# lijun9250lj/video-steganography-PCAMV

Hardware: AMD Instinct MI355X
Metric: 1080p macroblocks/s (embed on) (higher is better)
Workload: dtype u8

## Files before the change

### video-steganography-pcamv_amd/csrc/pcamv_common.h

```cpp
#ifndef PCAMV_COMMON_H
#define PCAMV_COMMON_H
#include <stddef.h>
#include <stdint.h>
#include "../../include/pcamv_gpu.h"
#include "pcamv_variant.h"

#ifdef PCAMV_HOST_EMU
#define PCAMV_DEV static inline
#define PCAMV_CONST static const
#else
#include <hip/hip_runtime.h>
#define PCAMV_DEV __device__ __forceinline__
#define PCAMV_CONST __device__ static const
#endif

#define PCAMV_PAD 32
#define PCAMV_CPAD 16
#define PCAMV_LSW 28
#define PCAMV_LROW 32
#define PCAMV_LSTRIPS(stride) (((stride) + PCAMV_LSW - 1) / PCAMV_LSW + 1)
#define PCAMV_LSTRIP_OF(x) (((uint32_t)(x) * 18725u) >> 19)
#define PCAMV_COST_MAX (1 << 28)
#define PCAMV_COST_MV_LEN (4 * 4 * 2048 + 1)
#define PCAMV_COST_MV_CENTRE (2 * 4 * 2048)
// ... 14 lines not shown
    uint8_t *luma[4];
    uint8_t *chroma[2];
    uint8_t *rec[3];
    int8_t *mb_type;
    int16_t *mv;
    int8_t *ref8;
    int16_t *mvr;
    const int16_t *prev_mv;
    const int8_t *prev_ref;
    int have_prev, tscale;
    pcamv_mb_t *rec_mb;
    int16_t *mvp_aux;
    const int16_t *cost_mv;
    int qp, chroma_qp, lambda, chroma_qp_offset;
    int me_method, me_range, subme, mv_range, b_chroma_me, b_fast_pskip, b_dct_decimate, b_cabac;
    unsigned inter;
    int embed;
    int q_mf[2][3], q_bias[2][3], dq_mf[3];
    int dq_mf_c[3];
    int lambda2_chroma;
    int *trace; int trace_mb;
    uint16_t *nnz;
    const int8_t *flip;
    const int *car_base;
    int b_mbrd, psy_rd, lambda2, ref_is_inter;
    int q_mf_i[3], q_bias_i[3];
    uint8_t *nb_nz;
    int16_t *nb_cbp;
    int16_t *nb_mvd;
    uint8_t *cabac;
    const uint8_t *cabac_init;
    const uint32_t *cabac_tab;
    uint32_t *dbg_hash;
    int rec_is_pass1;
    const uint8_t *mbflip;
    const struct FrameDev *self;
};

#ifdef PCAMV_HOST_EMU
#define FD(F) (F)
#else
#define PCAMV_AS4 __attribute__((address_space(4)))
PCAMV_DEV const PCAMV_AS4 FrameDev &fd_reload(const FrameDev &F)
{
    const uint64_t a = (uint64_t)F.self;
    uint32_t lo = (uint32_t)__builtin_amdgcn_readfirstlane((int)(uint32_t)a), hi = (uint32_t)__builtin_amdgcn_readfirstlane((int)(uint32_t)(a >> 32));
    asm volatile("" : "+s"(lo), "+s"(hi));
    return *(const PCAMV_AS4 FrameDev *)((uint64_t)hi << 32 | lo);
}
template <bool KEEP> PCAMV_DEV const auto &fd_pick(const FrameDev &F) { if constexpr (KEEP) return F; else return fd_reload(F); }
#ifdef PCAMV_NO_DESC_RELOAD
#define FD(F) (F)
#else
#define FD(F) fd_pick<PCAMV_RD_LO>(F)
#endif
#endif

PCAMV_DEV int nib32(unsigned k, int i) { return (int)((k >> (4 * i)) & 15u); }
PCAMV_DEV int nib64(unsigned long long k, int i) { return (int)((k >> (4 * i)) & 15ull); }
PCAMV_DEV int lg_w4_of(int ip) { return nib32(0x0011122u, ip); }
PCAMV_DEV int lg_h4_of(int ip) { return nib32(0x0101212u, ip); }
PCAMV_DEV int lg_nblk_of(int ip) { return nib32(0x0112334u, ip); }
PCAMV_DEV int pix_w_of(int ip) { return 4 << lg_w4_of(ip); }
PCAMV_DEV int pix_h_of(int ip) { return 4 << lg_h4_of(ip); }
PCAMV_DEV int blk_x_of(int idx) { return (idx & 1) | ((idx >> 1) & 2); }
PCAMV_DEV int blk_y_of(int idx) { return ((idx >> 1) & 1) | ((idx >> 2) & 2); }
PCAMV_DEV int scan8_of(int idx) { return SCAN8_0 + blk_x_of(idx) + 8 * blk_y_of(idx); }
PCAMV_DEV int clip3i(int v, int lo, int hi) { return v < lo ? lo : v > hi ? hi : v; }
PCAMV_DEV int iabs(int v) { return v < 0 ? -v : v; }
PCAMV_DEV int imin(int a, int b) { return a < b ? a : b; }
PCAMV_DEV int imax(int a, int b) { return a > b ? a : b; }
PCAMV_DEV int median3i(int a, int b, int c) { return imax(imin(a, b), imin(imax(a, b), c)); }
PCAMV_DEV int size_ue_of(unsigned v) { int n = 0; for (v++; v > 1; v >>= 1) n++; return 2 * n + 1; }
enum { I4_V, I4_H, I4_DC, I4_DDL, I4_DDR, I4_VR, I4_HD, I4_VL, I4_HU, I4_DC_LEFT, I4_DC_TOP, I4_DC_128 };

struct MBLocal {
    uint8_t fenc[24 * 16];
    int16_t cmv[48][2];
    int8_t cref[48];
    int16_t pskip_mv[2];
    int16_t mvr_own[2];
    int mb_x, mb_y, mb_xy;
    int mv_min[2], mv_max[2], mv_min_spel[2], mv_max_spel[2], mv_min_fpel[2], mv_max_fpel[2];
    int neighbour, type_left, type_top, type_topleft, type_topright;
    int i_type, i_partition;
    uint8_t sub_part[4];
    int b_skip_mc, cbp_luma, cbp_chroma;
    int nnz_mask;
    uint32_t cxy[64];
    int ccost[192];
    int slots[16];
    uint8_t recb[24 * 16];
    uint8_t recb0[24 * 16];
    uint8_t pred[24 * 16];
    union {
        struct {
            int16_t coef[24][16];
            int16_t cdc[2][4];
            int blk_nz[24], blk_score[24];
            int red[64];
        };
        uint8_t pred4[4][24 * 16];
    };
    int mvc16[9][2];
    int nbc[12];
    uint32_t win[(4 * 480 + 2 * 192) / 4];
    int win_x0, win_y0, win_cx0, win_cy0;
// ... 136 lines not shown
```

### video-steganography-pcamv_amd/csrc/pcamv_flow.hip.h

```cpp
#ifndef PCAMV_FLOW_HIP_H
#define PCAMV_FLOW_HIP_H
#include "pcamv_common.h"
#include "pcamv_prims_gpu.h"
#include "pcamv_mbkernels.h"
#include "pcamv_pass2.hip.h"

struct FlowDev {
    unsigned *ctr;
    unsigned *queue;
    int *dep;
    unsigned total, spin_limit;
    unsigned qbase[8], qcount[8];
    int n_gop, n_mb, mb_w, mb_h, fused, nq;
    int unit;
    int raster;
    int spec;
    unsigned *rdone;
};
#define RLX_AGENT __ATOMIC_RELAXED, __HIP_MEMORY_SCOPE_AGENT
#define FLOW_HEAD(q) (64 * (q))
#define FLOW_TAIL(q) (64 * (q) + 32)
#define FLOW_ERR 512
#define FLOW_CTR_WORDS 576
#define FLOW_RDONE_STRIDE 32
// ... 132 lines not shown
        if (MODE == 0 && (VARIANT & V_SPEC)) { if (!mbk_search_spec<VARIANT>(F, &L, Ap, x, y, fl, g, item)) break; }
        else if (MODE == 0) mbk_search<VARIANT>(F, &L, Ap, x, y);
        else {
            const int x0 = fl.unit * x, n = imin(fl.unit, F.mb_w - x0);
            p2_unit_load(F, Up, x0, y, n);
            for (int k = 0; k < n; k++) {
                if (mbk_pass2(F, &L, x0 + k, y, p2_pre(Up, k))) p2_put_mb(Up, &L, k);
                mbk_deblock_unit(F, Up, &L, k, x0 + k, y);
            }
            p2_unit_store(F, Up, x0, y, n);
        }
        PROF_ADD(MODE ? 14 : 1, t_s);
        const unsigned long long t_p = PROF_T();
        asm volatile("s_waitcnt vmcnt(0)" ::: "memory");
        if (MODE == 0 && (VARIANT & V_SPEC)) { }
        else if (lane == 0 && fl.raster) {
            if (xy + 1 < fl.n_mb) flow_done_one(fl, g & (fl.nq - 1), g * fl.n_mb + xy + 1, item + 1u);
        } else if (lane == 0) {
            const int base = g * fl.n_mb, q = g & (fl.nq - 1);
            if (x + 1 < fl.mb_w) flow_done_one(fl, q, base + xy + 1, item + 1u);
            if (y + 1 < fl.mb_h) {
                if (x >= 1) flow_done_one(fl, q, base + xy + fl.mb_w - 1, item + (unsigned)fl.mb_w - 1u);
                if (x == fl.mb_w - 1) flow_done_one(fl, q, base + xy + fl.mb_w, item + (unsigned)fl.mb_w);
            }
        }
        PROF_ADD(MODE ? 15 : 2, t_p);
        const unsigned long long t_r = PROF_T();
        if (MODE == 0 && fl.fused) {
            if (!fl.raster) {
                if (lane == 0) ticket = __hip_atomic_fetch_add(&fl.ctr[FLOW_HEAD(home)], 1u, RLX_AGENT);
                have_ticket = true;
            }
            mbk_rca_encode(F, &L, Ap, xy, 1, (VARIANT & V_RD) && F.b_mbrd);
        }
        PROF_ADD(3, t_r);
        if (MODE == 0) PROF_ADD(4, t_pop);
    }
    PROF_FLUSH();
}

#ifndef PCAMV_PROF
static_assert(sizeof(MBLocal) + sizeof(Analysis) <= PCAMV_WAVE_LDS_MAX, "the analysis kernels' LDS per wave (MBLocal + Analysis) no longer allows 16 waves per CU");
#endif

__device__ __forceinline__ bool diag_pos(const FrameDev &F, int d, int *x, int *y)
{
    int y_lo = d - (F.mb_w - 1); y_lo = y_lo > 0 ? (y_lo + 1) >> 1 : 0;
    *y = y_lo + (int)blockIdx.x; *x = d - 2 * *y;
    return *y < F.mb_h && *x >= 0 && *x < F.mb_w;
}

enum { P2D_PASS2 = 1, P2D_DEBLOCK = 2 };
void pcamv_launch_pass2_diag(int stages, unsigned blocks, unsigned gops, hipStream_t st, const FrameDev *dF, int d);
void pcamv_launch_flow_tesa(unsigned waves, hipStream_t st, const FrameDev *dF, const FlowDev &fl);
template <int BUILD> void pcamv_launch_flow_rd(unsigned waves, hipStream_t st, const FrameDev *dF, const FlowDev &fl);
template <int BUILD> int pcamv_flow_rd_waves_per_cu(void);
template <int BUILD> int pcamv_rd_prof_fetch(unsigned long long *out, int reset);
#endif
```

### video-steganography-pcamv_amd/csrc/pcamv_gpu.hip

```cpp
#include <hip/hip_runtime.h>
#include <math.h>
#include <stdarg.h>
#include <stdio.h>
#include <stdlib.h>
#include <string.h>
#include <new>
#include <vector>
#include "pcamv_planes.hip.h"
#include "pcamv_kernels.hip.h"
#include "pcamv_embed.hip.h"
#include "pcamv_message.hip.h"
#include "pcamv_slice.hip.h"
#include "pcamv_host_tables.h"
#include "pcamv_mvsyntax.h"
#include "pcamv_param_sets_host.h"
#include "pcamv_rd_select.h"
#include "pcamv_idr_defs.h"

#define PCAMV_ABI_VERSION 3
#define NEV 32
#define NRING 8
#define NKEV 16
#define PCAMV_TIMERS(X) \
    X(KT_ANALYSE, NULL) \
// ... 282 lines not shown
    for (int q = 0; q < 8; q++) {
        const unsigned ng = q < fl.nq ? ((unsigned)n + (unsigned)(fl.nq - 1 - q)) / (unsigned)fl.nq : 0u;
        fl.qbase[q] = qb; fl.qcount[q] = ng * (unsigned)fl.n_mb; qb += fl.qcount[q];
    }
}

static int batch_create_impl(pcamv_batch *b, pcamv_ctx_t *const *ctxs, int n)
{
    b->n = n; b->device = ctxs[0]->device; b->W = ctxs[0]->F.w; b->H = ctxs[0]->F.h;
    b->b_mbrd = ctxs[0]->F.b_mbrd;
    for (int i = 0; i < n; i++) b->b_tesa |= ctxs[i]->F.me_method == PCAMV_ME_TESA;
    b->ctx = (pcamv_ctx **)malloc(sizeof(pcamv_ctx *) * n);
    for (int i = 0; i < n; i++) b->ctx[i] = ctxs[i];
    const FrameDev &F = ctxs[0]->F;
    const int sub8x8 = (ctxs[0]->p.inter & PCAMV_ANALYSE_PSUB8x8) != 0;
    b->n_diag = F.mb_w + 2 * (F.mb_h - 1);
    b->max_diag = (F.mb_w + 1) / 2 < F.mb_h ? (F.mb_w + 1) / 2 : F.mb_h;
    b->slots_per_mb = sub8x8 ? 16 : 2;
    b->sched_flow = !env_is("PCAMV_SCHED", "diag") && F.n_mb <= 65535 && n <= 65535;
    { const int ns = env_int("PCAMV_STC_STATES", 2, 4, 0); b->stc_ns = ns == 2 || ns == 4 ? ns : (n >= 1024 ? 4 : 2); }
    b->sp_lds_cols = env_int("PCAMV_SLICE_LDS_COLS", 0, SP_LDS_COLS, SP_LDS_COLS);
    for (int k = 0; k < KT_N; k++) { b->kt[k].cap = k == KT_ANALYSE ? NEV : NKEV; b->kt[k].weight = 1; }
    if (!b->sched_flow) b->kt[KT_ANALYSE].weight = b->n_diag;
    HIPCHK(b, hipSetDevice(b->device));
    TRY(b->h_F.room(b, (size_t)n * NRING)); TRY(b->h_E.room(b, (size_t)n * NRING));
    TRY(b->d_F.room(b, (size_t)n * NRING)); TRY(b->d_E.room(b, (size_t)n * NRING));
    if (b->sched_flow) {
        const size_t total = (size_t)n * F.n_mb;
        TRY(b->d_flow.room(b, FLOW_CTR_WORDS + 2 * total + (size_t)FLOW_RDONE_STRIDE * n));
        FlowDev &fl = b->fl;
        fl.ctr = b->d_flow; fl.queue = b->d_flow + FLOW_CTR_WORDS; fl.dep = (int *)(b->d_flow + FLOW_CTR_WORDS + total);
        fl.rdone = b->d_flow + FLOW_CTR_WORDS + 2 * total; fl.spec = 0;
        fl.total = (unsigned)total; fl.spin_limit = 4u << 20;
        fl.n_gop = n; fl.n_mb = F.n_mb; fl.mb_w = F.mb_w; fl.mb_h = F.mb_h; fl.fused = 1; fl.unit = 1;
        fl.nq = env_is("PCAMV_FLOW_AFFINITY", "0") || n < 8 ? 1 : 8;
        flow_split_queues(fl, n);
        fl.raster = F.b_mbrd && (F.b_cabac || sub8x8);
        int per_cu = 0, n_cu = 0;
        HIPCHK(b, hipOccupancyMaxActiveBlocksPerMultiprocessor(&per_cu, k_analyse_flow, 64, 0));
        HIPCHK(b, hipDeviceGetAttribute(&n_cu, hipDeviceAttributeMultiprocessorCount, b->device));
        if (F.b_mbrd) {
            b->rd = &rd_builds[rd_select(n, n_cu, fl.raster, F.mb_w, sub8x8, b->b_tesa, getenv("PCAMV_RD_INSTANCE"), getenv("PCAMV_FLOW_SPEC"))];
            fl.spec = b->rd->spec != 0;
            per_cu = b->rd->waves_per_cu();
            if (per_cu < 0) return fail(b, PCAMV_EHIP, "the occupancy of the RD instance's build could not be read");
        }
        b->flow_waves = flow_wave_count(per_cu, n_cu, total);
        const int unit = env_int("PCAMV_PASS2_UNIT", 1, 8, n >= 256 ? 8 : 1);
        FlowDev &fl2 = b->fl2;
        fl2 = fl; fl2.unit = unit; fl2.raster = 0; fl2.spec = 0; fl2.mb_w = (F.mb_w + unit - 1) / unit; fl2.n_mb = fl2.mb_w * F.mb_h;
        fl2.total = (unsigned)n * (unsigned)fl2.n_mb;
        flow_split_queues(fl2, n);
        fl2.dep = (int *)(b->d_flow + FLOW_CTR_WORDS + fl2.total);
        HIPCHK(b, hipOccupancyMaxActiveBlocksPerMultiprocessor(&per_cu, k_pass2_deblock_flow, 64, 0));
        b->flow2_waves = flow_wave_count(per_cu, n_cu, fl2.total);
        HIPCHK(b, hipMemset(b->d_flow, 0, FLOW_CTR_WORDS * sizeof(unsigned)));
    }
    for (int i = 0; i < n; i++) if (ctxs[i]->n_member >= 16) return PCAMV_EINVAL;
    for (int i = 0; i < n; i++) ctxs[i]->member_of[ctxs[i]->n_member++] = b;
    for (int i = 0; i < n; i++)
        if ((ctxs[i]->F.me_method == PCAMV_ME_TESA || ctxs[i]->F.b_mbrd) && !b->sched_flow) return PCAMV_EUNSUP;
    return 0;
}
extern "C" int pcamv_gpu_batch_create(pcamv_ctx_t *const *ctxs, int n, pcamv_batch_t **out)
{
    if (!ctxs || n <= 0 || !out) return PCAMV_EINVAL;
    *out = NULL;
    for (int i = 0; i < n; i++)
        if (!ctxs[i] || ctxs[i]->device != ctxs[0]->device || ctxs[i]->F.w != ctxs[0]->F.w || ctxs[i]->F.h != ctxs[0]->F.h ||
            ctxs[i]->p.inter != ctxs[0]->p.inter || ctxs[i]->F.b_mbrd != ctxs[0]->F.b_mbrd || ctxs[i]->F.b_cabac != ctxs[0]->F.b_cabac) return PCAMV_EINVAL;
    pcamv_batch *b = new (std::nothrow) pcamv_batch();
    if (!b) return PCAMV_ENOMEM;
    const int rc = batch_create_impl(b, ctxs, n);
    if (rc) { pcamv_gpu_batch_destroy(b); return rc; }
    *out = b;
    return 0;
}
extern "C" const char *pcamv_gpu_batch_last_error(const pcamv_batch_t *b) { return b ? b->err : "no batch"; }
extern "C" int pcamv_gpu_batch_set_closed_loop(pcamv_batch_t *b, int on) { if (!b) return PCAMV_EINVAL; b->closed_loop = on != 0; return 0; }
static int flow_check(pcamv_batch *b);
extern "C" int pcamv_gpu_fetch_recon(pcamv_ctx_t *c, uint8_t *const planes[3])
{
    if (!c || !planes) return PCAMV_EINVAL;
    HIPCHK(c, hipSetDevice(c->device));
    HIPCHK(c, hipDeviceSynchronize());
    TRY(on_behalf(c, c->last, flow_check(c->last)));
    const size_t ysz = (size_t)c->F.w * c->F.h;
    for (int i = 0; i < 3; i++)
        if (planes[i]) HIPCHK(c, hipMemcpy(planes[i], c->F.rec[i], i ? ysz / 4 : ysz, hipMemcpyDeviceToHost));
    return 0;
}
extern "C" int pcamv_gpu_recon_device(pcamv_ctx_t *c, void *planes[3])
{
    if (!c || !planes) return PCAMV_EINVAL;
    for (int i = 0; i < 3; i++) planes[i] = c->F.rec[i];
    return 0;
}
static const char *dominant_kernel(const pcamv_batch *b)
{
    if (!b || !b->sched_flow) return "k_search_diag";
    if (b->b_mbrd) return "k_analyse_flow_rd";
    if (b->b_tesa) return "k_analyse_flow_tesa";
    return "k_analyse_flow";
}
extern "C" const char *pcamv_gpu_batch_dominant_kernel(const pcamv_batch_t *b) { return dominant_kernel(b); }
static const char *kt_name(const pcamv_batch *b, int k)
{
// ... 276 lines not shown
    for (int i = 0; i < b->n; i++) {
        pcamv_ctx *c = b->ctx[i];
        if ((what & ST_ANALYSE) && c->prev_internal) {
            const int wr = !c->last_field;
            c->F.mv = wr ? c->d_mv_b : c->d_mv; c->F.ref8 = wr ? c->d_ref8_b : c->d_ref8;
            c->F.prev_mv = wr ? c->d_mv : c->d_mv_b; c->F.prev_ref = wr ? c->d_ref8 : c->d_ref8_b;
        }
        if (what & ST_ANALYSE) c->last_field = c->F.mv == c->d_mv_b;
        if (what & ST_ANALYSE) c->rec_pristine = 1;
        if (what & ST_PASS2) pass2_takes_rec(c);
        else c->F.rec_is_pass1 = 0;
    }
    const FrameDev *dF; const EmbedDev *dE; int slot;
    TRY(batch_push_descs(b, st, &dF, &dE, &slot));
    const FrameDev &F = b->ctx[0]->F;
    const unsigned G = (unsigned)b->n;
    if (what & ST_PLANES) {
        dim3 g(((F.stride + PCAMV_LSW - 1) / PCAMV_LSW + 7) / 8, (F.lines + HP_ROWS - 1) / HP_ROWS, G);
        hipLaunchKernelGGL(k_hpel, g, dim3(HP_THREADS), 0, st, dF);
        dim3 gc((F.cstride / 16 * CP_ROWS + CP_THREADS - 1) / CP_THREADS, (F.clines + CP_ROWS - 1) / CP_ROWS, 2 * G);
        hipLaunchKernelGGL(k_chroma_pad, gc, dim3(CP_THREADS), 0, st, dF);
    }
    if (what & ST_ANALYSE) {
        for (int i = 0; i < b->n; i++) b->ctx[i]->last = b;
        if (b->sched_flow) {
            hipLaunchKernelGGL(k_flow_init, dim3((b->fl.total + 255) / 256), dim3(256), 0, st, b->fl);
            timed(b, KT_ANALYSE, st, [&] {
                if (b->b_mbrd) b->rd->launch((unsigned)b->flow_waves, st, dF, b->fl);
                else if (b->b_tesa) pcamv_launch_flow_tesa((unsigned)b->flow_waves, st, dF, b->fl);
                else hipLaunchKernelGGL(k_analyse_flow, dim3(b->flow_waves), dim3(64), 0, st, dF, b->fl);
            });
        } else {
            timed(b, KT_ANALYSE, st, [&] {
                diag_launch(b->n_diag, F, [&](int cnt, int d) { hipLaunchKernelGGL(k_search_diag<0>, dim3(cnt, G), dim3(64), 0, st, dF, d); });
            });
            hipLaunchKernelGGL(k_rca, dim3(F.n_mb * b->slots_per_mb, G), dim3(64), 0, st, dF, b->slots_per_mb);
            hipLaunchKernelGGL(k_encode, dim3(F.n_mb, G), dim3(64), 0, st, dF);
        }
    }
    if ((what & ST_EMBED) && b->d_msg) {
        timed_kernel(b, KT_MESSAGE_COUNT, st, k_message_count, dim3(G), dim3(256), dE, b->d_mtx_m);
        timed_kernel(b, KT_MESSAGE_PLAN, st, k_message_plan, dim3(1), dim3(MSG_PLAN_THREADS), b->d_mtx_m, (const int *)NULL, b->n, 1, PCAMV_MSG_NO_CAP, b->d_mtx, b->d_mtx_at, dE);
    }
    if (what & ST_EMBED) {
        timed_kernel(b, KT_EMBED_PREPARE, st, k_embed_prepare, dim3(G), dim3(1024), dE);
        if (b->stc_ns == 4) hipLaunchKernelGGL(k_stc_forward<4>, dim3(G), dim3(256), 0, st, dE);
        else hipLaunchKernelGGL(k_stc_forward<2>, dim3(G), dim3(512), 0, st, dE);
        hipLaunchKernelGGL(k_stc_backward, dim3(G), dim3(64), 0, st, dE);
        hipLaunchKernelGGL(k_mb_flips, dim3((F.n_mb + 255) / 256, G), dim3(256), 0, st, dE);
    }
    if (what & ST_PASS2) {
        if (b->sched_flow) {
            hipLaunchKernelGGL(k_flow_init, dim3((b->fl2.total + 255) / 256), dim3(256), 0, st, b->fl2);
            hipLaunchKernelGGL(k_pass2_deblock_flow, dim3(b->flow2_waves), dim3(64), 0, st, dF, b->fl2);
        } else {
            diag_launch(b->n_diag, F, [&](int cnt, int d) { pcamv_launch_pass2_diag(P2D_PASS2 | P2D_DEBLOCK, cnt, G, st, dF, d); });
        }
    }
    TRY(launched(b));
    return ring_release(b, b->ring, slot, st);
}
static int flow_check(pcamv_batch *b)
{
    if (!b || !b->sched_flow) return 0;
    unsigned bad = 0;
    HIPCHK(b, hipMemcpy(&bad, b->fl.ctr + FLOW_ERR, sizeof(bad), hipMemcpyDeviceToHost));
    if (bad) {
        hipMemset(b->fl.ctr + FLOW_ERR, 0, sizeof(unsigned));
        for (int i = 0; i < b->n; i++) if (b->ctx[i]) drop_rec_reuse(b->ctx[i]);
        return fail(b, PCAMV_EHIP, "dataflow kernel: queue wait timed out (results of the last step are incomplete)");
    }
    return 0;
}
static int ctx_launch(pcamv_ctx *c, int what) { return on_behalf(c, c->self, batch_launch(c->self, what, c->stream)); }

extern "C" int pcamv_gpu_set_ref(pcamv_ctx_t *c, const uint8_t *const plane[3], const int stride[3], const int16_t *prev_mv, const int8_t *prev_ref)
{
    if (!c || !plane || !stride) return PCAMV_EINVAL;
    HIPCHK(c, hipSetDevice(c->device));
    for (int i = 0; i < 3; i++) {
        int w = c->F.w >> !!i, h = c->F.h >> !!i;
        HIPCHK(c, hipMemcpy2D(c->d_raw[i], w, plane[i], stride[i], w, h, hipMemcpyHostToDevice));
        c->F.raw[i] = c->d_raw[i];
    }
    c->F.have_prev = prev_mv != NULL && prev_ref != NULL && c->p.i_tscale != 0;
    c->F.ref_is_inter = prev_mv != NULL && prev_ref != NULL;
    c->prev_internal = 0;
    c->F.mv = c->d_mv; c->F.ref8 = c->d_ref8;
    c->F.prev_mv = c->d_prev_mv; c->F.prev_ref = c->d_prev_ref;
    if (c->F.have_prev) {
        HIPCHK(c, hipMemcpy(c->d_prev_mv, prev_mv, (size_t)c->F.n_mb * 64, hipMemcpyHostToDevice));
        HIPCHK(c, hipMemcpy(c->d_prev_ref, prev_ref, (size_t)c->F.n_mb * 4, hipMemcpyHostToDevice));
    }
    drop_rec_reuse(c);
    TRY(ctx_launch(c, ST_PLANES));
    HIPCHK(c, hipStreamSynchronize(c->stream));
    return 0;
}
extern "C" int pcamv_gpu_set_ref_device(pcamv_ctx_t *c, const void *y, const void *u, const void *v, const void *prev_mv, const void *prev_ref)
{
    if (!c || !y || !u || !v) return PCAMV_EINVAL;
    c->F.have_prev = prev_mv != NULL && prev_ref != NULL && c->p.i_tscale != 0;
    c->F.ref_is_inter = prev_mv != NULL && prev_ref != NULL;
    c->prev_internal = prev_mv == PCAMV_PREV_FIELD_INTERNAL;
    if (c->F.have_prev && !c->prev_internal) { c->F.prev_mv = (const int16_t *)prev_mv; c->F.prev_ref = (const int8_t *)prev_ref; c->F.mv = c->d_mv; c->F.ref8 = c->d_ref8; }
    c->F.raw[0] = (const uint8_t *)y; c->F.raw[1] = (const uint8_t *)u; c->F.raw[2] = (const uint8_t *)v;
    return 0;
// ... 2237 lines not shown
```

### video-steganography-pcamv_amd/csrc/pcamv_kernels.hip.h

```cpp
#ifndef PCAMV_KERNELS_HIP_H
#define PCAMV_KERNELS_HIP_H
#include "pcamv_flow.hip.h"

template <int VARIANT>
__global__ void __launch_bounds__(64) k_search_diag(const FrameDev *__restrict__ Fs, int d)
{
    __shared__ MBLocal L;
    __shared__ Analysis A;
    const FrameDev F = Fs[blockIdx.y];
    int x, y;
    if (!diag_pos(F, d, &x, &y)) return;
    mbk_search<VARIANT>(F, &L, &A, x, y);
}
static __global__ void __launch_bounds__(64) k_rca(const FrameDev *__restrict__ Fs, int slots_per_mb)
{
    __shared__ MBLocal L;
    __shared__ Analysis A;
    const FrameDev F = Fs[blockIdx.y];
    if (!F.embed) return;
    int xy = blockIdx.x / slots_per_mb, k = blockIdx.x - xy * slots_per_mb;
    if (xy >= F.n_mb) return;
    mbk_rca(F, &L, &A, xy, k);
}
static __global__ void __launch_bounds__(64) k_encode(const FrameDev *__restrict__ Fs)
{
    __shared__ MBLocal L;
    __shared__ Analysis A;
    const FrameDev F = Fs[blockIdx.y];
    if ((int)blockIdx.x >= F.n_mb) return;
    mbk_encode(F, &L, &A, blockIdx.x);
}

static __global__ void __launch_bounds__(256) k_flow_init(FlowDev fl)
{
    unsigned i = blockIdx.x * 256u + threadIdx.x;
    if (i >= fl.total) return;
    int xy = (int)(i % (unsigned)fl.n_mb), x = xy % fl.mb_w, y = xy / fl.mb_w;
    fl.dep[i] = fl.raster ? (xy > 0) : (x > 0) + (y > 0);
    int q = 0;
    while (q + 1 < fl.nq && i >= fl.qbase[q + 1]) q++;
    const unsigned k = i - fl.qbase[q], ngop_q = fl.qcount[q] / (unsigned)fl.n_mb;
    fl.queue[i] = k < ngop_q ? ((k * (unsigned)fl.nq + (unsigned)q) << 16) + 1u : 0u;
    if (i < 8) { fl.ctr[FLOW_HEAD(i)] = 0u; fl.ctr[FLOW_TAIL(i)] = fl.qcount[i] / (unsigned)fl.n_mb; }
    if (fl.spec && i < (unsigned)fl.n_gop) fl.rdone[FLOW_RDONE_STRIDE * i] = 0u;
}
static __global__ void __launch_bounds__(64, PCAMV_FLOW_OCC) k_analyse_flow(const FrameDev *__restrict__ Fs, FlowDev fl)
{
    __shared__ MBLocal L;
    __shared__ Analysis A;
    flow_loop<0, 0>(Fs, fl, L, &A, nullptr);
}

#ifndef PCAMV_PASS2_OCC
#define PCAMV_PASS2_OCC 4
#endif
static __global__ void __launch_bounds__(64, PCAMV_PASS2_OCC) k_pass2_deblock_flow(const FrameDev *__restrict__ Fs, FlowDev fl)
{
    __shared__ __attribute__((aligned(16))) uint8_t Lraw[PCAMV_PASS2_LDS];
    __shared__ __attribute__((aligned(16))) P2Unit U;
    flow_loop<1, 0>(Fs, fl, *reinterpret_cast<MBLocal *>(Lraw), nullptr, &U);
}

static __global__ void __launch_bounds__(64) k_block_costs(const FrameDev *__restrict__ Fs, const int *__restrict__ req, int *__restrict__ out)
{
    __shared__ MBLocal L;
    const FrameDev F = Fs[0];
    const int *r = req + 8 * blockIdx.x;
    L.mb_x = r[0]; L.mb_y = r[1]; L.mb_xy = r[1] * F.mb_w + r[0];
    prim_load_fenc(F, &L);
    PCAMV_WAVE_SYNC();
    const int mflag = (r[7] & 1 ? EV_SATD : 0) | EV_NOMV;
    if (r[7] & 2) {
        if (LANE() == 0) {
            L.cxy[0] = CAND_PACK(r[5], r[6]); L.cxy[1] = CAND_PACK(r[5] + 1, r[6] - 1);
            L.cxy[2] = CAND_PACK(r[5] - 2, r[6] + 3); L.cxy[3] = CAND_PACK(r[5] + 3, r[6] + 2);
        }
        prim_eval_list(F, &L, L.fenc, r[2], r[3], r[4], 4, mflag, 0, 0);
        if (LANE() == 0) { out[3 * blockIdx.x] = L.ccost[1]; out[3 * blockIdx.x + 1] = L.ccost[2]; out[3 * blockIdx.x + 2] = L.ccost[3]; }
        return;
    }
    if (LANE() == 0) { L.cxy[0] = CAND_PACK(r[5], r[6]); L.ccost[64] = 0; L.ccost[128] = 0; }
    prim_eval_list(F, &L, L.fenc, r[2], r[3], r[4], 1, mflag | EV_CHROMA | EV_PROBE, 0, 0);
    if (LANE() == 0) { out[3 * blockIdx.x] = L.ccost[0]; out[3 * blockIdx.x + 1] = L.ccost[64]; out[3 * blockIdx.x + 2] = L.ccost[128]; }
}

static __global__ void __launch_bounds__(64) k_rd_probe(const FrameDev *__restrict__ Fs, const uint8_t *__restrict__ req, int *__restrict__ out)
{
    __shared__ MBLocal L;
    const FrameDev F = Fs[0];
    const int lane = LANE();
    const uint8_t *r = req + 1024 * (size_t)blockIdx.x;
    int *o = out + 32 * blockIdx.x;
    for (int i = lane; i < 96; i += 64) { ((uint32_t *)L.fenc)[i] = ((const uint32_t *)r)[i]; ((uint32_t *)L.pred)[i] = ((const uint32_t *)(r + 384))[i]; }
    for (int i = lane; i < 84; i += 64) ((uint8_t *)L.ib_top)[i] = r[768 + i];
    if (lane < 48) ((uint8_t *)L.ib_left)[lane] = r[852 + lane];
    const int avail = *(const int *)(r + 900);
    if (lane == 0) { L.mb_x = L.mb_y = L.mb_xy = 0; L.neighbour = (avail & 1 ? NB_LEFT : 0) | (avail & 2 ? NB_TOP | NB_TOPRIGHT : 0) | (avail == 3 ? NB_TOPLEFT : 0); }
    PCAMV_WAVE_SYNC();
    FrameDev F0 = F;
    F0.psy_rd = 0;
    const int ssd0 = prim_ssd_mb(F0, &L);
    prim_fenc_complexity(F, &L);
    const int ssd1 = prim_ssd_mb(F, &L);
    int h4, h8;
    prim_hadamard_ac16(L.pred, lane, &h4, &h8);
    if (lane == 0) { o[0] = ssd0; o[1] = ssd1; o[2] = h4; o[3] = h8; o[4] = L.fenc_satd_sum; o[5] = L.fenc_sa8d_sum; }
    prim_intra16_satd(F, &L, avail);
    if (lane < 4) o[6 + lane] = L.ccost[lane];
    PCAMV_WAVE_SYNC();
    prim_intra8c_satd(F, &L, avail);
    if (lane < 4) o[10 + lane] = L.ccost[lane];
    PCAMV_WAVE_SYNC();
    prim_intra4_init(&L);
// ... 6 lines not shown
```

### video-steganography-pcamv_amd/csrc/pcamv_planes.hip.h

```cpp
#ifndef PCAMV_PLANES_HIP_H
#define PCAMV_PLANES_HIP_H
#include "pcamv_common.h"
#include "pcamv_prims_gpu.h"

typedef uint32_t u32x4 __attribute__((ext_vector_type(4)));
typedef __attribute__((address_space(1))) u32x4 *gp128w;
typedef __attribute__((address_space(1))) uint32_t *gp32w;
typedef const __attribute__((address_space(1))) uint32_t *gp32;
#define CP_ROWS 4
#define CP_THREADS 256
static __global__ void __launch_bounds__(CP_THREADS) k_chroma_pad(const FrameDev *__restrict__ Fs)
{
    const FrameDev &F = Fs[blockIdx.z >> 1];
    const int pl = blockIdx.z & 1;
    const uint8_t *__restrict__ src = F.raw[1 + pl];
    uint8_t *__restrict__ dst = F.chroma_base[pl];
    const int w = F.w >> 1, h = F.h >> 1, cstride = F.cstride, clines = F.clines;
    const int per_row = cstride >> 4;
    const int i = blockIdx.x * CP_THREADS + threadIdx.x;
    const int y = blockIdx.y * CP_ROWS + i / per_row, x = 16 * (i % per_row);
    if (i >= per_row * CP_ROWS || y >= clines) return;
    const uint8_t *rowp = src + (size_t)clip3i(y - PCAMV_CPAD, 0, h - 1) * w;
    const bool aligned = ((uintptr_t)src & 3) == 0;
    uint32_t v[4];
#pragma unroll
    for (int k = 0; k < 4; k++) {
        const int gx = x + 4 * k - PCAMV_CPAD;
        if (gx < 0 || gx >= w) v[k] = rowp[gx < 0 ? 0 : w - 1] * 0x01010101u;
        else if (aligned) v[k] = *(const uint32_t *)(rowp + gx);
        else v[k] = rowp[gx] | rowp[gx + 1] << 8 | rowp[gx + 2] << 16 | (uint32_t)rowp[gx + 3] << 24;
    }
    *(gp128w)(dst + (size_t)y * cstride + x) = u32x4{v[0], v[1], v[2], v[3]};
}

#define HP_ROWS 16
#define HP_THREADS 64
#define HP_TILE 40
__device__ __forceinline__ void hpel_load_row(const uint8_t *__restrict__ rowp, int eg0, int W, bool fast, uint32_t d[3])
{
    if (fast) {
        const gp32 q = (gp32)(rowp + eg0 - 4);
        d[0] = q[0]; d[1] = q[1]; d[2] = q[2];
    } else {
#pragma unroll
        for (int i = 0; i < 3; i++) {
            uint32_t v = 0;
#pragma unroll
            for (int b = 0; b < 4; b++) v |= (uint32_t)rowp[clip3i(eg0 - 4 + 4 * i + b, 0, W - 1)] << (8 * b);
            d[i] = v;
        }
    }
}
static __global__ void __launch_bounds__(HP_THREADS) k_hpel(const FrameDev *__restrict__ Fs)
{
    __shared__ uint32_t tile[4][8][HP_TILE];
    const FrameDev &F = Fs[blockIdx.z];
    const uint8_t *__restrict__ src = F.raw[0];
    uint8_t *__restrict__ planes = F.luma_base;
    const int W = F.w, H = F.h, stride = F.stride, lines = F.lines;
    const int t = threadIdx.x >> 3, d = threadIdx.x & 7;
    const int strip = blockIdx.x * 8 + t, yb = blockIdx.y * HP_ROWS;
    if (strip * PCAMV_LSW >= stride) return;
    const int x0 = strip * PCAMV_LSW + 4 * d;
    const int gx = x0 - PCAMV_PAD, eg0 = clip3i(gx, -4, W);
    const int rep = gx < -4 ? 0 : gx > W ? 3 : -1;
    const bool fast = eg0 >= 4 && eg0 + 8 <= W && ((uintptr_t)src & 3) == 0;
    const size_t psz = (size_t)F.plane_size;
    uint8_t *const line0 = planes + (size_t)strip * PCAMV_LROW * (size_t)lines + 16 * d;
    const bool raster = F.luma_raster && d < 7 && x0 < stride;
    uint32_t w[6][3];
    uint32_t of = 0, oh = 0, ov = 0, oc = 0;
    int ey_prev = 0;
    for (int y = yb; y < yb + HP_ROWS && y < lines; y++) {
        const int ey = clip3i(y - PCAMV_PAD, -8, H + 7);
        if (y == yb || ey != ey_prev) {
            if (y == yb) {
#pragma unroll
                for (int k = 0; k < 5; k++) hpel_load_row(src + (size_t)clip3i(ey - 2 + k, 0, H - 1) * W, eg0, W, fast, w[k]);
            } else {
#pragma unroll
                for (int k = 0; k < 5; k++) { w[k][0] = w[k + 1][0]; w[k][1] = w[k + 1][1]; w[k][2] = w[k + 1][2]; }
            }
            hpel_load_row(src + (size_t)clip3i(ey + 3, 0, H - 1) * W, eg0, W, fast, w[5]);
            ey_prev = ey;
            int v[9], b2[9];
#pragma unroll
            for (int j = 0; j < 9; j++) {
                const int q = (j + 2) >> 2, sh = 8 * ((j + 2) & 3);
#define HPB(k) ((int)(w[k][q] >> sh & 255))
                v[j] = HPB(0) + HPB(5) - 5 * (HPB(1) + HPB(4)) + 20 * (HPB(2) + HPB(3));
                b2[j] = HPB(2);
#undef HPB
            }
            of = w[2][1]; oh = ov = oc = 0;
#pragma unroll
            for (int k = 0; k < 4; k++) {
                const int th = b2[k] + b2[k + 5] - 5 * (b2[k + 1] + b2[k + 4]) + 20 * (b2[k + 2] + b2[k + 3]);
                const int tc = v[k] + v[k + 5] - 5 * (v[k + 1] + v[k + 4]) + 20 * (v[k + 2] + v[k + 3]);
                oh |= clamp_u8((th + 16) >> 5) << (8 * k);
                ov |= clamp_u8((v[k + 2] + 16) >> 5) << (8 * k);
                oc |= clamp_u8((tc + 512) >> 10) << (8 * k);
            }
            if (rep >= 0) {
                const int sh = 8 * rep;
                of = (of >> sh & 255) * 0x01010101u; oh = (oh >> sh & 255) * 0x01010101u;
                ov = (ov >> sh & 255) * 0x01010101u; oc = (oc >> sh & 255) * 0x01010101u;
            }
        }
        if (raster) *(gp32w)(F.luma_raster + (size_t)y * stride + x0) = of;
        const int r = y & 3;
        tile[0][t][8 * r + d] = of; tile[1][t][8 * r + d] = oh; tile[2][t][8 * r + d] = ov; tile[3][t][8 * r + d] = oc;
        if (r == 3) {
            PCAMV_WAVE_SYNC();
            u32x4 ln[4];
#pragma unroll
            for (int k = 0; k < 4; k++) ln[k] = *(const u32x4 *)&tile[k][t][4 * d];
            PCAMV_WAVE_SYNC();
            uint8_t *const o = line0 + (size_t)(y - 3) * PCAMV_LROW;
#pragma unroll
            for (int k = 0; k < 4; k++) *(gp128w)(o + k * psz) = ln[k];
        }
    }
}
#endif
```

### video-steganography-pcamv_amd/pcamv_amd/api.py

```python
import ctypes as C
import os
import subprocess

import numpy as np

_PKG = os.path.dirname(os.path.dirname(os.path.abspath(__file__)))
_CSRC = os.path.join(_PKG, "csrc")

ME_NAMES = {"dia": 0, "hex": 1, "umh": 2, "esa": 3, "tesa": 4}
P_L0, P_8x8, P_SKIP = 4, 5, 6
I4x4, PSUB16x16, PSUB8x8 = 0x01, 0x10, 0x20


class PcamvError(RuntimeError):
    pass


class Params(C.Structure):
    _fields_ = [("i_width", C.c_int32), ("i_height", C.c_int32), ("i_me_method", C.c_int32),
                ("i_me_range", C.c_int32), ("i_subpel_refine", C.c_int32), ("i_mv_range", C.c_int32),
                ("b_chroma_me", C.c_int32), ("b_fast_pskip", C.c_int32), ("b_dct_decimate", C.c_int32),
                ("b_cabac", C.c_int32), ("inter", C.c_uint32), ("i_chroma_qp_offset", C.c_int32),
                ("i_luma_deadzone", C.c_int32 * 2), ("i_tscale", C.c_int32), ("i_psy_rd", C.c_int32)]

# ... 45 lines not shown
    p.i_luma_deadzone[0], p.i_luma_deadzone[1] = 21, 11
    p.i_tscale = 256
    p._f_psy_rd, p._chroma_qp_offset = 1.0, 0
    return _validate(p)


def param_parse(p, name, value):
    name = name.lstrip("-").replace("_", "-")
    if name == "me":
        if value not in ME_NAMES:
            raise PcamvError(f"invalid value for me: {value}")
        p.i_me_method = ME_NAMES[value]
    elif name in ("merange", "me-range"):
        p.i_me_range = int(value)
    elif name in ("subme", "subq"):
        p.i_subpel_refine = int(value)
    elif name == "mvrange":
        p.i_mv_range = int(value)
    elif name in ("partitions", "analyse"):
        v = 0
        toks = [t.strip() for t in str(value).split(",")]
        if "none" in toks:
            v = 0
        if "all" in toks or "i4x4" in toks:
            v |= I4x4
        if "all" in toks or "p8x8" in toks:
            v |= PSUB16x16
        if "all" in toks or "p4x4" in toks:
            v |= PSUB8x8
        if not (v & PSUB16x16):
            v &= ~PSUB8x8
        p.inter = v
    elif name == "no-chroma-me":
        p.b_chroma_me = 0
    elif name == "no-fast-pskip":
        p.b_fast_pskip = 0
    elif name == "no-dct-decimate":
        p.b_dct_decimate = 0
    elif name == "no-cabac":
        p.b_cabac = 0
    elif name == "chroma-qp-offset":
        p._chroma_qp_offset = int(value)
    elif name == "psy-rd":
        p._f_psy_rd = float(str(value).split(":")[0])
    else:
        raise PcamvError(f"unknown option: {name}")
    return _validate(p)


def lib_path():
    return os.environ.get("PCAMV_GPU_LIB") or os.path.join(_PKG, "libpcamv_gpu.so")


UNITS = ("pcamv_gpu", "pcamv_pass2_diag", "pcamv_slice_write", "pcamv_slice_write_cavlc", "pcamv_idr", "pcamv_tesa", "pcamv_rd", "pcamv_rd_lo", "pcamv_rd_spec", "pcamv_rd_spec2", "pcamv_rd_spec4", "pcamv_rd_tesa")


def build_library(force=False):
    out = lib_path()
    srcs = [os.path.join(_CSRC, f) for f in sorted(os.listdir(_CSRC)) if not f.endswith(".o")]
    srcs.append(os.path.join(os.path.dirname(_PKG), "include", "pcamv_gpu.h"))
    if not force and os.path.exists(out) and all(os.path.getmtime(out) >= os.path.getmtime(s) for s in srcs):
        return out
    flags = ["--offload-arch=gfx950", "-O3", "-ffp-contract=off", "-fPIC", "-std=c++17", "-Wno-unused-value", "-Wno-unused-result"]
    objs, procs = [], []
    for unit in UNITS:
        obj = os.path.join(_CSRC, unit + ".o")
        objs.append(obj)
        procs.append(subprocess.Popen(["hipcc", *flags, "-c", "-o", obj, os.path.join(_CSRC, unit + ".hip")]))
    rcs = [p.wait() for p in procs]
    if any(rcs):
        raise subprocess.CalledProcessError(max(rcs), "hipcc -c (csrc/*.hip)")
    subprocess.check_call(["hipcc", "--offload-arch=gfx950", "-fPIC", "-shared", "-o", out, *objs])
    for obj in objs:
        os.remove(obj)
    return out


_lib = None


def load_library():
    global _lib
    if _lib is None:
        path = lib_path()
        if not os.path.exists(path):
            raise PcamvError(f"{path} is missing: run __graft_entry__.build() (hipcc). There is no CPU fallback.")
        _lib = C.CDLL(path)
        _lib.pcamv_gpu_last_error.restype = C.c_char_p
        _lib.pcamv_gpu_last_error.argtypes = [C.c_void_p]
        _lib.pcamv_gpu_close.restype = None
        _lib.pcamv_gpu_close.argtypes = [C.c_void_p]
    return _lib


def _p(a):
    return a.ctypes.data_as(C.c_void_p) if a is not None else None


def parse_pslice_cabac(slice_data, mb_w, mb_h, qp):
    data = np.frombuffer(bytes(slice_data), np.uint8)
    mbs = np.zeros(mb_w * mb_h, MB_DTYPE)
    lib = load_library()
    lib.pcamv_gpu_parse_pslice_cabac.argtypes = [C.c_void_p, C.c_size_t, C.c_int, C.c_int, C.c_int, C.c_void_p]
    rc = lib.pcamv_gpu_parse_pslice_cabac(_p(data), len(data), mb_w, mb_h, qp, _p(mbs))
    if rc:
        raise PcamvError(f"pcamv_gpu_parse_pslice_cabac failed: {rc}")
    return mbs
# ... 1395 lines not shown
```

Measured before the change: 26.47 million.

## Split pass2 flow kernel into own unit and vectorise half-pel interpolation

Moves the pass-2 deblock flow kernel into its own compilation unit, built so that the frame descriptor is kept in registers rather than reloaded through scalar loads. Separately, the half-pel filter kernel is rewritten to use packed 16-bit lanes, byte permutes and dot-product instructions. It also gains a fully unrolled fast path with a rotating six-row window for interior tiles. The aim is fewer instructions per pixel and lower descriptor reload overhead, at the cost of possibly higher register pressure and a separate occupancy query.

```diff
diff --git a/video-steganography-pcamv_amd/csrc/pcamv_common.h b/video-steganography-pcamv_amd/csrc/pcamv_common.h
--- a/video-steganography-pcamv_amd/csrc/pcamv_common.h
+++ b/video-steganography-pcamv_amd/csrc/pcamv_common.h
@@ -90,7 +90,10 @@
 #ifdef PCAMV_NO_DESC_RELOAD
 #define FD(F) (F)
 #else
-#define FD(F) fd_pick<PCAMV_RD_LO>(F)
+#ifndef PCAMV_FD_KEEP
+#define PCAMV_FD_KEEP 0
+#endif
+#define FD(F) fd_pick<(PCAMV_RD_LO) || (PCAMV_FD_KEEP)>(F)
 #endif
 #endif
 
diff --git a/video-steganography-pcamv_amd/csrc/pcamv_flow.hip.h b/video-steganography-pcamv_amd/csrc/pcamv_flow.hip.h
--- a/video-steganography-pcamv_amd/csrc/pcamv_flow.hip.h
+++ b/video-steganography-pcamv_amd/csrc/pcamv_flow.hip.h
@@ -208,6 +208,8 @@
 
 enum { P2D_PASS2 = 1, P2D_DEBLOCK = 2 };
 void pcamv_launch_pass2_diag(int stages, unsigned blocks, unsigned gops, hipStream_t st, const FrameDev *dF, int d);
+void pcamv_launch_pass2_flow(unsigned waves, hipStream_t st, const FrameDev *dF, const FlowDev &fl);
+int pcamv_pass2_flow_waves_per_cu(void);
 void pcamv_launch_flow_tesa(unsigned waves, hipStream_t st, const FrameDev *dF, const FlowDev &fl);
 template <int BUILD> void pcamv_launch_flow_rd(unsigned waves, hipStream_t st, const FrameDev *dF, const FlowDev &fl);
 template <int BUILD> int pcamv_flow_rd_waves_per_cu(void);
diff --git a/video-steganography-pcamv_amd/csrc/pcamv_gpu.hip b/video-steganography-pcamv_amd/csrc/pcamv_gpu.hip
--- a/video-steganography-pcamv_amd/csrc/pcamv_gpu.hip
+++ b/video-steganography-pcamv_amd/csrc/pcamv_gpu.hip
@@ -358,7 +358,8 @@
         fl2.total = (unsigned)n * (unsigned)fl2.n_mb;
         flow_split_queues(fl2, n);
         fl2.dep = (int *)(b->d_flow + FLOW_CTR_WORDS + fl2.total);
-        HIPCHK(b, hipOccupancyMaxActiveBlocksPerMultiprocessor(&per_cu, k_pass2_deblock_flow, 64, 0));
+        per_cu = pcamv_pass2_flow_waves_per_cu();
+        if (per_cu < 0) return fail(b, PCAMV_EHIP, "the occupancy of the second-pass kernel could not be read");
         b->flow2_waves = flow_wave_count(per_cu, n_cu, fl2.total);
         HIPCHK(b, hipMemset(b->d_flow, 0, FLOW_CTR_WORDS * sizeof(unsigned)));
     }
@@ -741,7 +742,7 @@
     if (what & ST_PASS2) {
         if (b->sched_flow) {
             hipLaunchKernelGGL(k_flow_init, dim3((b->fl2.total + 255) / 256), dim3(256), 0, st, b->fl2);
-            hipLaunchKernelGGL(k_pass2_deblock_flow, dim3(b->flow2_waves), dim3(64), 0, st, dF, b->fl2);
+            pcamv_launch_pass2_flow((unsigned)b->flow2_waves, st, dF, b->fl2);
         } else {
             diag_launch(b->n_diag, F, [&](int cnt, int d) { pcamv_launch_pass2_diag(P2D_PASS2 | P2D_DEBLOCK, cnt, G, st, dF, d); });
         }
diff --git a/video-steganography-pcamv_amd/csrc/pcamv_kernels.hip.h b/video-steganography-pcamv_amd/csrc/pcamv_kernels.hip.h
--- a/video-steganography-pcamv_amd/csrc/pcamv_kernels.hip.h
+++ b/video-steganography-pcamv_amd/csrc/pcamv_kernels.hip.h
@@ -49,16 +49,6 @@
     __shared__ MBLocal L;
     __shared__ Analysis A;
     flow_loop<0, 0>(Fs, fl, L, &A, nullptr);
-}
-
-#ifndef PCAMV_PASS2_OCC
-#define PCAMV_PASS2_OCC 4
-#endif
-static __global__ void __launch_bounds__(64, PCAMV_PASS2_OCC) k_pass2_deblock_flow(const FrameDev *__restrict__ Fs, FlowDev fl)
-{
-    __shared__ __attribute__((aligned(16))) uint8_t Lraw[PCAMV_PASS2_LDS];
-    __shared__ __attribute__((aligned(16))) P2Unit U;
-    flow_loop<1, 0>(Fs, fl, *reinterpret_cast<MBLocal *>(Lraw), nullptr, &U);
 }
 
 static __global__ void __launch_bounds__(64) k_block_costs(const FrameDev *__restrict__ Fs, const int *__restrict__ req, int *__restrict__ out)
diff --git a/video-steganography-pcamv_amd/csrc/pcamv_pass2_flow.hip b/video-steganography-pcamv_amd/csrc/pcamv_pass2_flow.hip
--- /dev/null
+++ b/video-steganography-pcamv_amd/csrc/pcamv_pass2_flow.hip
@@ -0,0 +1,25 @@
+#include <hip/hip_runtime.h>
+#include <stdint.h>
+#define PCAMV_FD_KEEP 1
+#include "pcamv_flow.hip.h"
+
+#ifndef PCAMV_PASS2_OCC
+#define PCAMV_PASS2_OCC 4
+#endif
+static __global__ void __launch_bounds__(64, PCAMV_PASS2_OCC) k_pass2_deblock_flow(const FrameDev *__restrict__ Fs, FlowDev fl)
+{
+    __shared__ __attribute__((aligned(16))) uint8_t Lraw[PCAMV_PASS2_LDS];
+    __shared__ __attribute__((aligned(16))) P2Unit U;
+    flow_loop<1, 0>(Fs, fl, *reinterpret_cast<MBLocal *>(Lraw), nullptr, &U);
+}
+
+void pcamv_launch_pass2_flow(unsigned waves, hipStream_t st, const FrameDev *dF, const FlowDev &fl)
+{
+    hipLaunchKernelGGL(k_pass2_deblock_flow, dim3(waves), dim3(64), 0, st, dF, fl);
+}
+int pcamv_pass2_flow_waves_per_cu(void)
+{
+    int per_cu = 0;
+    if (hipOccupancyMaxActiveBlocksPerMultiprocessor(&per_cu, k_pass2_deblock_flow, 64, 0) != hipSuccess) return -1;
+    return per_cu;
+}
diff --git a/video-steganography-pcamv_amd/csrc/pcamv_planes.hip.h b/video-steganography-pcamv_amd/csrc/pcamv_planes.hip.h
--- a/video-steganography-pcamv_amd/csrc/pcamv_planes.hip.h
+++ b/video-steganography-pcamv_amd/csrc/pcamv_planes.hip.h
@@ -51,6 +51,46 @@
         }
     }
 }
+struct HpRow { v2s p[6]; };
+__device__ __forceinline__ void hpel_unpack(const uint32_t d[3], HpRow &r)
+{
+#pragma unroll
+    for (int i = 0; i < 3; i++) {
+        r.p[2 * i] = as_v2s(__builtin_amdgcn_perm(0u, d[i], 0x0c010c00u));
+        r.p[2 * i + 1] = as_v2s(__builtin_amdgcn_perm(0u, d[i], 0x0c030c02u));
+    }
+}
+__device__ __forceinline__ v2s hp_tap6(v2s a, v2s b, v2s c, v2s d, v2s e, v2s f) { return ((a + f) + (c + d) * (short)20) - (b + e) * (short)5; }
+__device__ __forceinline__ v2s hp_odd(v2s lo, v2s hi) { return as_v2s(__builtin_amdgcn_alignbit(as_u32(hi), as_u32(lo), 16)); }
+__device__ __forceinline__ v2s hp_clamp(v2s v) { return __builtin_elementwise_min(__builtin_elementwise_max(v, (v2s)(short)0), (v2s)(short)255); }
+__device__ __forceinline__ v2s hp_round5(v2s v) { return hp_clamp((v + (short)16) >> (short)5); }
+#define HP_PACK 0x06040200u
+__device__ __forceinline__ uint32_t hp_pack_u8(v2s lo, v2s hi, uint32_t sel) { return __builtin_amdgcn_perm(as_u32(hi), as_u32(lo), sel); }
+__device__ __forceinline__ int hp_centre(v2s a, v2s b, v2s c)
+{
+    int t = __builtin_amdgcn_sdot2(a, (v2s){1, -5}, 512, false);
+    t = __builtin_amdgcn_sdot2(b, (v2s){20, 20}, t, false);
+    t = __builtin_amdgcn_sdot2(c, (v2s){-5, 1}, t, false) >> 10;
+    asm volatile("" : "+v"(t));
+    return t;
+}
+__device__ __forceinline__ void hpel_row_out(const HpRow &r0, const HpRow &r1, const HpRow &r2, const HpRow &r3, const HpRow &r4, const HpRow &r5,
+                                             uint32_t sel, uint32_t &of, uint32_t &oh, uint32_t &ov, uint32_t &oc)
+{
+    v2s V[6];
+#pragma unroll
+    for (int i = 1; i < 6; i++) V[i] = hp_tap6(r0.p[i], r1.p[i], r2.p[i], r3.p[i], r4.p[i], r5.p[i]);
+    const v2s *p = r2.p;
+    const v2s q1 = hp_odd(p[1], p[2]), q2 = hp_odd(p[2], p[3]), q3 = hp_odd(p[3], p[4]), q4 = hp_odd(p[4], p[5]);
+    const v2s h01 = hp_tap6(p[1], q1, p[2], q2, p[3], q3), h23 = hp_tap6(p[2], q2, p[3], q3, p[4], q4);
+    const v2s w1 = hp_odd(V[1], V[2]), w2 = hp_odd(V[2], V[3]), w3 = hp_odd(V[3], V[4]), w4 = hp_odd(V[4], V[5]);
+    const v2s c01 = {(short)hp_centre(V[1], V[2], V[3]), (short)hp_centre(w1, w2, w3)};
+    const v2s c23 = {(short)hp_centre(V[2], V[3], V[4]), (short)hp_centre(w2, w3, w4)};
+    of = hp_pack_u8(p[2], p[3], sel);
+    oh = hp_pack_u8(hp_round5(h01), hp_round5(h23), sel);
+    ov = hp_pack_u8(hp_round5(V[2]), hp_round5(V[3]), sel);
+    oc = hp_pack_u8(hp_clamp(c01), hp_clamp(c23), sel);
+}
 static __global__ void __launch_bounds__(HP_THREADS) k_hpel(const FrameDev *__restrict__ Fs)
 {
     __shared__ uint32_t tile[4][8][HP_TILE];
@@ -64,49 +104,14 @@
     const int x0 = strip * PCAMV_LSW + 4 * d;
     const int gx = x0 - PCAMV_PAD, eg0 = clip3i(gx, -4, W);
     const int rep = gx < -4 ? 0 : gx > W ? 3 : -1;
+    const uint32_t sel = rep < 0 ? HP_PACK : 2u * (uint32_t)rep * 0x01010101u;
     const bool fast = eg0 >= 4 && eg0 + 8 <= W && ((uintptr_t)src & 3) == 0;
     const size_t psz = (size_t)F.plane_size;
     uint8_t *const line0 = planes + (size_t)strip * PCAMV_LROW * (size_t)lines + 16 * d;
     const bool raster = F.luma_raster && d < 7 && x0 < stride;
-    uint32_t w[6][3];
+    HpRow w[6];
     uint32_t of = 0, oh = 0, ov = 0, oc = 0;
-    int ey_prev = 0;
-    for (int y = yb; y < yb + HP_ROWS && y < lines; y++) {
-        const int ey = clip3i(y - PCAMV_PAD, -8, H + 7);
-        if (y == yb || ey != ey_prev) {
-            if (y == yb) {
-#pragma unroll
-                for (int k = 0; k < 5; k++) hpel_load_row(src + (size_t)clip3i(ey - 2 + k, 0, H - 1) * W, eg0, W, fast, w[k]);
-            } else {
-#pragma unroll
-                for (int k = 0; k < 5; k++) { w[k][0] = w[k + 1][0]; w[k][1] = w[k + 1][1]; w[k][2] = w[k + 1][2]; }
-            }
-            hpel_load_row(src + (size_t)clip3i(ey + 3, 0, H - 1) * W, eg0, W, fast, w[5]);
-            ey_prev = ey;
-            int v[9], b2[9];
-#pragma unroll
-            for (int j = 0; j < 9; j++) {
-                const int q = (j + 2) >> 2, sh = 8 * ((j + 2) & 3);
-#define HPB(k) ((int)(w[k][q] >> sh & 255))
-                v[j] = HPB(0) + HPB(5) - 5 * (HPB(1) + HPB(4)) + 20 * (HPB(2) + HPB(3));
-                b2[j] = HPB(2);
-#undef HPB
-            }
-            of = w[2][1]; oh = ov = oc = 0;
-#pragma unroll
-            for (int k = 0; k < 4; k++) {
-                const int th = b2[k] + b2[k + 5] - 5 * (b2[k + 1] + b2[k + 4]) + 20 * (b2[k + 2] + b2[k + 3]);
-                const int tc = v[k] + v[k + 5] - 5 * (v[k + 1] + v[k + 4]) + 20 * (v[k + 2] + v[k + 3]);
-                oh |= clamp_u8((th + 16) >> 5) << (8 * k);
-                ov |= clamp_u8((v[k + 2] + 16) >> 5) << (8 * k);
-                oc |= clamp_u8((tc + 512) >> 10) << (8 * k);
-            }
-            if (rep >= 0) {
-                const int sh = 8 * rep;
-                of = (of >> sh & 255) * 0x01010101u; oh = (oh >> sh & 255) * 0x01010101u;
-                ov = (ov >> sh & 255) * 0x01010101u; oc = (oc >> sh & 255) * 0x01010101u;
-            }
-        }
+    auto put = [&](int y) {
         if (raster) *(gp32w)(F.luma_raster + (size_t)y * stride + x0) = of;
         const int r = y & 3;
         tile[0][t][8 * r + d] = of; tile[1][t][8 * r + d] = oh; tile[2][t][8 * r + d] = ov; tile[3][t][8 * r + d] = oc;
@@ -120,6 +125,44 @@
 #pragma unroll
             for (int k = 0; k < 4; k++) *(gp128w)(o + k * psz) = ln[k];
         }
+    };
+    auto load_raw = [&](int sy, uint32_t raw[3]) { hpel_load_row(src + (size_t)clip3i(sy, 0, H - 1) * W, eg0, W, fast, raw); };
+    auto load = [&](int sy, HpRow &r) {
+        uint32_t raw[3];
+        load_raw(sy, raw);
+        hpel_unpack(raw, r);
+    };
+    const int ey0 = yb - PCAMV_PAD;
+    if (ey0 >= -8 && ey0 + HP_ROWS - 1 <= H + 7 && yb + HP_ROWS <= lines) {
+        uint32_t raw[3];
+#pragma unroll
+        for (int k = 0; k < 5; k++) load(ey0 - 2 + k, w[k]);
+        load_raw(ey0 + 3, raw);
+#pragma unroll
+        for (int i = 0; i < HP_ROWS; i++) {
+            hpel_unpack(raw, w[(i + 5) % 6]);
+            if (i + 1 < HP_ROWS) load_raw(ey0 + i + 4, raw);
+            hpel_row_out(w[i % 6], w[(i + 1) % 6], w[(i + 2) % 6], w[(i + 3) % 6], w[(i + 4) % 6], w[(i + 5) % 6], sel, of, oh, ov, oc);
+            put(yb + i);
+        }
+        return;
+    }
+    int ey_prev = 0;
+    for (int y = yb; y < yb + HP_ROWS && y < lines; y++) {
+        const int ey = clip3i(y - PCAMV_PAD, -8, H + 7);
+        if (y == yb || ey != ey_prev) {
+            if (y == yb) {
+#pragma unroll
+                for (int k = 0; k < 5; k++) load(ey - 2 + k, w[k]);
+            } else {
+#pragma unroll
+                for (int k = 0; k < 5; k++) w[k] = w[k + 1];
+            }
+            load(ey + 3, w[5]);
+            ey_prev = ey;
+            hpel_row_out(w[0], w[1], w[2], w[3], w[4], w[5], sel, of, oh, ov, oc);
+        }
+        put(y);
     }
 }
 #endif
diff --git a/video-steganography-pcamv_amd/pcamv_amd/api.py b/video-steganography-pcamv_amd/pcamv_amd/api.py
--- a/video-steganography-pcamv_amd/pcamv_amd/api.py
+++ b/video-steganography-pcamv_amd/pcamv_amd/api.py
@@ -121,7 +121,7 @@
     return os.environ.get("PCAMV_GPU_LIB") or os.path.join(_PKG, "libpcamv_gpu.so")
 
 
-UNITS = ("pcamv_gpu", "pcamv_pass2_diag", "pcamv_slice_write", "pcamv_slice_write_cavlc", "pcamv_idr", "pcamv_tesa", "pcamv_rd", "pcamv_rd_lo", "pcamv_rd_spec", "pcamv_rd_spec2", "pcamv_rd_spec4", "pcamv_rd_tesa")
+UNITS = ("pcamv_gpu", "pcamv_pass2_diag", "pcamv_pass2_flow", "pcamv_slice_write", "pcamv_slice_write_cavlc", "pcamv_idr", "pcamv_tesa", "pcamv_rd", "pcamv_rd_lo", "pcamv_rd_spec", "pcamv_rd_spec2", "pcamv_rd_spec4", "pcamv_rd_tesa")
 
 
 def build_library(force=False):
```

New measurement: 26.63 million, median of 6. About the same (+0.6%).
